# r-papso/carca-replication

Measured on AMD Instinct MI355X. Metric: scored users/sec (1+100 candidates), CARCA eval forward, higher is better.
Workload: dtype f32

## Files before the change

### carca_replication_amd/_lib.py

```python
from __future__ import annotations

import ctypes as C
import hashlib
import os
import shutil
import subprocess
import threading

_HERE = os.path.dirname(os.path.abspath(__file__))
_CSRC = os.path.join(_HERE, "csrc")
_INCLUDE = os.path.join(os.path.dirname(_HERE), "include")
LIB_PATH = os.path.join(_HERE, "libcarca_hip.so")
_STAMP = LIB_PATH + ".srchash"
SOURCES = ["api.hip", "gemm.hip", "gemm_wgrad.hip", "gemm_split.hip", "gemm_stream.hip", "wgrad_cu.hip", "decoders.hip", "batch_build.hip", "embed.hip", "sa_block.hip", "sa_eval.hip", "cross_score.hip", "cross_stream.hip", "loss_metrics.hip", "backward.hip", "block_bwd.hip", "row_chain.hip", "optim.hip", "recommend.hip", "rank.hip", "knn_catalogue.hip",
           "catalogue_xent.hip", "feat_dedup.hip", "sampled_xent.hip", "sampled_bce.hip", "similar_items.hip"]
HEADERS = ["carca_common.h", "gemm_host.h", "attn_common.h", "gemm_epilogue.h", "cross_fold.h", "recommend_common.h", "catalogue_select.h",
           "catalogue_sweep.h", "xent_tile.h", "xent_stage.h"]

MAX_SEGS = 4
MAX_GROUPS = 3
MAX_L = 64

_lock = threading.Lock()
_lib = None
# ... 294 lines not shown
    "carca_sa_block_eval": (_i, [_fp, _i, _fp, _fp, _i, _i, _i, _i, _i, C.POINTER(SaWeights), _i, _i, _fp]),
    "carca_cross_score_fwd": (_i, [_fp, _i, _fp, _fp, C.POINTER(TargetGroup), _i, _i, _i, _i, _i, _i,
                                   C.POINTER(CaWeights), _i, _i, C.POINTER(CaSave), C.POINTER(Dropout), _fp]),
    "carca_dropout_fwd": (_i, [_fp, _i, _i, _i, C.POINTER(Dropout), _fp, _fp]),
    "carca_mask_mul": (_i, [_fp, _i, _fp, _i, _f, _fp, _i, _i, _i, _i, _fp]),
    "carca_layernorm_bwd": (_i, [_fp, _i, _fp, _i, _fp, _i, _i, _fp, _i, _fp, _i, _i, _fp, _fp, _fp]),
    "carca_embed_scatter": (_i, [_fp, _i, _fp, _i, _i, _f, _fp, _fp]),
    "carca_colsum": (_i, [_fp, _i, _i, _i, _fp, _fp, _i, _fp, _fp]),
    "carca_sa_attn_bwd": (_i, [_fp, _fp, _fp, _fp, _i, _fp, _fp, _fp, _fp, _i, _i, _i, _i, _fp, _f, _fp]),
    "carca_cross_attn_bwd": (_i, [_fp, _fp, _fp, C.POINTER(CrossBwdGroup), _i, _fp, _fp, _fp, _fp, _i, _i, _i, _i, _i,
                                  _f, _fp]),
    "carca_unpack_grads": (_i, [C.POINTER(PackDesc), _i, _i, _fp]),
    "carca_forward": (_i, [C.POINTER(ForwardDesc), C.POINTER(_fp), _fp]),
    "carca_event_create": (_i, [C.POINTER(_fp)]),
    "carca_event_destroy": (_i, [_fp]),
    "carca_event_elapsed_ms": (_i, [_fp, _fp, C.POINTER(C.c_float)]),
    "carca_stream_wait_event": (_i, [_fp, _fp]),
    "carca_bce_fwd": (_i, [_fp, _fp, _fp, _i, _f, _fp, _fp, _fp, _fp, _fp]),
    "carca_rank_metrics": (_i, [_fp, _i, _i, _i, _fp, _fp, _fp, _fp]),
    "carca_eval_metrics": (_i, [_fp, _fp, _fp, _i, _i, _i, _f, _fp, _fp]),
    "carca_layernorm_fwd": (_i, [_fp, _i, _fp, _i, _i, _i, _fp, _fp, _fp]),
    "carca_dot_score_fwd": (_i, [_fp, _i, _fp, _i, _fp, _i, _i, _i, _i, _i, _i, _fp]),
    "carca_dot_score_bwd": (_i, [_fp, _i, _fp, _i, _fp, _fp, _fp, _i, _fp, _i, _i, _i, _i, _i, _i, _i, _fp]),
    "carca_slot_decay_scale": (_i, [_fp, _i, _fp, _i, _i, _i, _i, _f, _fp]),
    "carca_l2norm_fwd": (_i, [_fp, _i, _fp, _i, _i, _i, _fp]),
    "carca_l2norm_bwd": (_i, [_fp, _i, _fp, _i, _fp, _i, _i, _i, _fp]),
    "carca_add_positions": (_i, [_fp, _i, _fp, _fp, _i, _i, _i, _i, _fp]),
    "carca_mha_core": (_i, [_fp, _i, _fp, _fp, _i, _fp, _fp, _i, _i, _i, _i, _i, _i, _i, _fp, _i, _fp, _fp]),
    "carca_mha_core_bwd": (_i, [_fp, _i, _fp, _fp, _i, _fp, _fp, _i, _i, _i, _i, _i, _i, _i, _fp, _i, _fp, _fp, _fp, _fp,
                                _fp]),
    "carca_gemm_rows_log": (_i, [C.c_char_p, _i]),
    "carca_feat_dedup_rows_multiplied": (C.c_longlong, []),
    "carca_feat_dedup_rows_computed": (C.c_longlong, []),
    "carca_feat_cache_arm": (_i, [C.POINTER(FeatCache)]),
    "carca_get_tuning": (_i, [_i]),
    "carca_mha_core_drop": (_i, [_fp, _i, _fp, _fp, _i, _fp, _fp, _i, _i, _i, _i, _i, _i, _i, _fp, _i, _fp, C.POINTER(Dropout),
                                 _fp, _fp]),
    "carca_mha_core_bwd_drop": (_i, [_fp, _i, _fp, _fp, _i, _fp, _fp, _i, _i, _i, _i, _i, _i, _i, _fp, _i, _fp, _fp, _fp, _fp,
                                     _fp, C.c_float, _fp]),
    "carca_knn_score": (_i, [_fp, C.c_int64, _fp, C.c_int64, _fp, _fp, _i, _fp, _i, _i, _i, _i, _fp]),
    "carca_sa_block_bwd_workspace": (C.c_size_t, [_i, _i, _i, _i]),
    "carca_sa_block_bwd": (_i, [C.POINTER(SaBwdDesc), C.POINTER(WgradDesc), C.POINTER(_i), _fp]),
    "carca_cross_score_bwd_workspace": (C.c_size_t, [_i, _i, _i, _i, C.POINTER(C.c_int32), _i]),
    "carca_cross_score_bwd": (_i, [C.POINTER(CrossBwdDesc), C.POINTER(WgradDesc), C.POINTER(_i), _fp]),
    "carca_embed_bwd_workspace": (C.c_size_t, [C.POINTER(C.c_int32), _i, _i, _i]),
    "carca_embed_bwd": (_i, [C.POINTER(EmbedBwdDesc), _fp]),
    "carca_early_event_recorded": (_i, []),
    "carca_adam_step": (_i, [C.POINTER(AdamTensor), _i, C.c_double, C.c_double, C.c_double, C.c_double, C.c_double, _i,
                        _fp]),
    "carca_mark_rows": (_i, [_fp, C.c_int64, _fp, C.c_int64, _fp]),
    "carca_zero_rows": (_i, [_fp, C.c_int64, _i, C.POINTER(_fp), C.POINTER(C.c_int64), _i, _fp]),
    "carca_concat_ids": (_i, [C.POINTER(_fp), C.POINTER(C.c_int64), _i, _fp, _fp]),
    "carca_build_eval_batch": (_i, [_fp, _fp, _fp, _fp, _i, _i, _i, _i, _i, _i, _i, _i, C.c_uint64, _fp, _fp, _fp, _fp, _fp,
                                    _fp]),
    "carca_recommend": (_i, [C.POINTER(RecommendDesc), _fp]),
    "carca_rank_items": (_i, [C.POINTER(RankDesc), _fp]),
    "carca_recommend_among": (_i, [C.POINTER(RecommendDesc), C.POINTER(Candidates), _fp]),
    "carca_rank_items_among": (_i, [C.POINTER(RankDesc), C.POINTER(Candidates), _fp]),
    "carca_knn_recommend": (_i, [C.POINTER(KnnRecommendDesc), _fp]),
    "carca_knn_rank_items": (_i, [C.POINTER(KnnRankDesc), _fp]),
    "carca_row_rnorm": (_i, [_fp, _i, _i, _i, _fp, _fp]),
    "carca_similar_items": (_i, [C.POINTER(SimilarDesc), C.POINTER(Candidates), _fp]),
    "carca_catalogue_xent_fwd": (_i, [C.POINTER(CatalogueXentDesc), _fp]),
    "carca_catalogue_xent_bwd": (_i, [C.POINTER(CatalogueXentDesc), _fp]),
    "carca_sampled_xent_fwd": (_i, [C.POINTER(SampledXentDesc), _fp]),
    "carca_sampled_xent_bwd": (_i, [C.POINTER(SampledXentDesc), _fp]),
# ... 48 lines not shown
```

### carca_replication_amd/csrc/carca_common.h

```cpp
#pragma once
#include <hip/hip_runtime.h>
#include <stdint.h>

#include "../../include/carca_hip.h"

typedef float f32x4 __attribute__((ext_vector_type(4)));
typedef float f32x16 __attribute__((ext_vector_type(16)));
typedef float f32x4_u __attribute__((ext_vector_type(4), aligned(4)));

#define CARCA_WAVE 64

typedef unsigned u32x4 __attribute__((ext_vector_type(4)));
__device__ __forceinline__ __amdgpu_buffer_rsrc_t carca_rsrc(const void* base) {
  return __builtin_amdgcn_make_buffer_rsrc(const_cast<void*>(base), 0, -1, 0x00020000);
}
__device__ __forceinline__ f32x4 gload4(const float* base, int elem_off) {
  const u32x4 v = __builtin_amdgcn_raw_buffer_load_b128(carca_rsrc(base), elem_off * 4, 0, 0);
  f32x4 f = {__uint_as_float(v[0]), __uint_as_float(v[1]), __uint_as_float(v[2]), __uint_as_float(v[3])};
  return f;
}
__device__ __forceinline__ f32x4 gload4s(const float* base, int lane_elem_off, int uniform_elem_off) {
  const u32x4 v = __builtin_amdgcn_raw_buffer_load_b128(carca_rsrc(base), lane_elem_off * 4, uniform_elem_off * 4, 0);
  f32x4 f = {__uint_as_float(v[0]), __uint_as_float(v[1]), __uint_as_float(v[2]), __uint_as_float(v[3])};
  return f;
// ... 130 lines not shown
      for (int i = 0; i < RIF; ++i) v[i] = c < ga.d ? src[i][c] : 0.f;
#pragma unroll
      for (int i = 0; i < RIF; ++i)
        if (c < ga.d && row0 + i < ga.total_rows) ga.zq[(size_t)(row0 + i) * ga.ldz + c] = v[i] * ga.scale;
    }
  }
}

template <int BYTES>
__device__ __forceinline__ void carca_warm_kernargs() {
  typedef const __attribute__((address_space(4))) int* karg_ptr;
  karg_ptr ka = (karg_ptr)__builtin_amdgcn_kernarg_segment_ptr();
  int w = 0;
#pragma unroll
  for (int i = 0; i < (BYTES + 63) / 64; ++i) w ^= ka[i * 16];
  asm volatile("" ::"s"(w));
}

enum { CARCA_TUNE_GEMM_VARIANT = 0, CARCA_TUNE_ATTN_VARIANT = 1, CARCA_TUNE_WGRAD_SLOTS = 2,
       CARCA_TUNE_WGRAD_PLAIN_STORE = 3,
       CARCA_TUNE_WGRAD_MIN_CHUNKS = 4,
       CARCA_TUNE_WGRAD_GROUP_SLOTS = 5,
       CARCA_TUNE_N96S_DIAG = 5,
       CARCA_TUNE_ROUND1_PATHS = 6,
       CARCA_TUNE_SCORE_LAYOUT = 7,
       CARCA_TUNE_DETERMINISTIC = 8,
       CARCA_TUNE_STAMPS = 9, CARCA_TUNE_CU_CAP = 10, CARCA_TUNE_SK_DON = 11, CARCA_TUNE_SK_SPIN_LOG2 = 12,
       CARCA_TUNE_SK_WITHHOLD = 13, CARCA_TUNE_XS_OPT = 14, CARCA_TUNE_DIAG = 15, CARCA_TUNE_SPLIT_GEMM = 16,
       CARCA_TUNE_SKC_OV_TEAM = 17,
       CARCA_TUNE_SKC_OV_LONE = 18,
       CARCA_TUNE_SKC_MIN_STEPS = 19,
       CARCA_TUNE_FEAT_DEDUP = 20,
       CARCA_TUNE_FEAT_CACHE = 21,
       CARCA_TUNE_COUNT = 24 };
enum {
  CARCA_GV_AUTO = 0,
  CARCA_GV_TILED = 1,
  CARCA_GV_PER_CU = 2,
  CARCA_GV_PER_CU_STAMPS = 3,
  CARCA_GV_NO_BUFFER_LOADS = 4,
  CARCA_GV_WGRAD_TILED = 5,
  CARCA_GV_NO_GROUP = 6,
  CARCA_GV_PER_CU_128 = 7,
  CARCA_GV_NO_PASSENGER = 8,
  CARCA_GV_WIDE64 = 9,
  CARCA_GV_WIDE64_PF2 = 10,
  CARCA_GV_N96 = 11,
  CARCA_GV_NO_N96 = 12,
  CARCA_GV_WGRAD_EQUAL_ITEMS = 13,
  CARCA_GV_WGRAD_ATOMIC_FLUSH = 14,
  CARCA_GV_NO_STREAM_K = 15,
  CARCA_GV_WGRAD_FLAT_GROUPS = 16,
  CARCA_GV_GATHER_ROW_PER_WAVE = 18,
  CARCA_GV_OWN_GATHER = 19,
  CARCA_GV_WPART_ATOMICS = 19,
  CARCA_GV_SPLIT_NO_DMA = 21,
  CARCA_GV_WGRAD_NO_COMPACT = 22,
  CARCA_GV_SK_EVERY_ROW = 23,
  CARCA_GV_NO_CUS = 24,
  CARCA_GV_CUS = 25,
  CARCA_GV_NO_N96S = 26,
  CARCA_GV_N96S = 27,
  CARCA_GV_NO_STREAM_K_NO_PASSENGER = 158,
};
int carca_tuning(int key);
int carca_num_cus();
bool carca_stream_capturing(hipStream_t stream);
void* carca_stream_scratch(hipStream_t stream, int tag, size_t bytes, size_t zero_bytes = 0, bool* fresh = nullptr);
enum { CARCA_SCRATCH_SK = 1, CARCA_SCRATCH_WPART = 2, CARCA_SCRATCH_WTAB = 3, CARCA_SCRATCH_SPLITW = 4, CARCA_SCRATCH_SKC = 5,
       CARCA_SCRATCH_SKC_PART = 6, CARCA_SCRATCH_RECOMMEND = 7, CARCA_SCRATCH_RANK = 8,
       CARCA_SCRATCH_KNN = 9, CARCA_SCRATCH_DEDUP_HASH = 10, CARCA_SCRATCH_DEDUP = 11, CARCA_SCRATCH_SIMILAR = 12 };
void* carca_capture_alloc(hipStream_t stream, size_t bytes, bool host_mapped, void** device_view, size_t zero_bytes = 0);
void carca_arm_launch_events(void* start, void* stop);
bool carca_take_launch_events(hipEvent_t* start, hipEvent_t* stop);
bool carca_take_feat_cache(CarcaFeatCache* out);
struct CarcaGemmDesc;
void carca_rows_log(const char* kernel, const CarcaGemmDesc* d, int grid);
int carca_gemm_rows_split_try(const CarcaGemmDesc* desc, hipStream_t stream);
int carca_gemm_rows_stream_try(const CarcaGemmDesc* desc, bool fits32, hipStream_t stream);
int carca_gemm_rows_n96s_try(const CarcaGemmDesc* desc, bool fits32, hipStream_t stream);
int carca_gemm_rows_passenger(const CarcaGemmDesc* desc, const CarcaGatherArgs* ga, int* rode, void* stream);
struct CarcaDedupRun {
  CarcaGemmDesc d;
  int nseg, R, vec, vec2, hbits;
  int row0[CARCA_MAX_SEGS + 1];
  unsigned hmask;
  int* key;
  unsigned* val;
  int *slot, *rep, *flag;
  float* P;
  float* wcb;
  int ldp;
  CarcaFeatCache cache;
  int *need, *pub, *cnt;
};
int carca_feat_dedup_prepare(const CarcaGemmDesc* desc, hipStream_t stream, CarcaDedupRun* run);
int carca_feat_dedup_plan(const CarcaDedupRun* run, hipStream_t stream, hipEvent_t start);
int carca_feat_dedup_expand(const CarcaDedupRun* run, hipStream_t stream, hipEvent_t stop);
int carca_gemm_rows_feat_dedup(const CarcaGemmDesc* desc, void* stream);
int* carca_kernel_error_word();
struct CarcaRowSeg;
int carca_embed_joint_ztab(const CarcaRowSeg* segs, int nseg, int d, int g, const float* joint_w, const float* joint_b,
                           const float* pos, const float* zq, int ld_e, const float* z_table, int ld_z_table, void* stream);
int carca_embed_scatter_segs(const float* const* dz, int ld_dz, const int32_t* const* ids, const int* rows, int nseg,
                             int d, float scale, float* d_items, void* stream);
int carca_sa_ffn_chain_bwd(const float* dy, const float* h1, const float* r, const float* w2_t, const float* w1_t,
                           const float* ln2_w, int rows, int d, int dpi, int residual, float* dh1pre, float* dr,
                           float* g_ln2_w, float* g_ln2_b, void* stream);
int carca_sa_input_chain_bwd(const float* dqh, const float* dkh, const float* dvh, const float* dr, const float* x_in,
                             const float* wq_t, const float* wk_t, const float* wv_t, const float* ln1_w, int rows, int d,
                             int dpi, int residual, float* dx, float* g_ln1_w, float* g_ln1_b, void* stream);
unsigned long long* carca_debug_buffer();
#define CARCA_CHECK_ARG(cond, ...)            \
  do {                                        \
    if (!(cond)) {                            \
      carca_set_error(__VA_ARGS__);           \
      return CARCA_ERR_BADARG;                \
    }                                         \
  } while (0)
#define CARCA_CHECK_SUPPORTED(cond, ...)      \
  do {                                        \
    if (!(cond)) {                            \
      carca_set_error(__VA_ARGS__);           \
      return CARCA_ERR_UNSUPPORTED;           \
    }                                         \
  } while (0)
#define CARCA_LAUNCH_CHECK()                                               \
// ... 8 lines not shown
```

### carca_replication_amd/csrc/feat_dedup.hip

```cpp
#include <hip/hip_ext.h>

#include <vector>

#include "carca_common.h"
#include "../../include/carca_hip.h"

namespace {

constexpr int EXP_ROWS = 16;
constexpr int EXP_MAX_N = 1024;
constexpr int EXP_MAX_K1 = 8;
constexpr int EXP_WB4 = ((EXP_MAX_K1 + 1) * EXP_MAX_N / 4 + 255) / 256;
__host__ __device__ inline int exp_wb_floats(int K1, int N) { return ((K1 + 1) * N + 3) / 4 * 4; }

__device__ __forceinline__ int dd_seg(const CarcaDedupRun& a, int g) {
  int s = 0;
#pragma unroll
  for (int i = 1; i < CARCA_MAX_SEGS; ++i)
    if (i < a.nseg && g >= a.row0[i]) s = i;
  return s;
}
__device__ __forceinline__ const float* dd_a0_row(const CarcaDedupRun& a, int s, int r) {
  const CarcaGemmSeg& sg = a.d.seg[s];
  if (sg.a0_gather) return sg.a0 + (size_t)sg.ids[r] * a.d.lda0;
  if (sg.a0_bstride) return sg.a0 + (size_t)(r / sg.T) * sg.a0_bstride + (size_t)(r % sg.T) * a.d.lda0;
  return sg.a0 + (size_t)r * a.d.lda0;
}

__global__ __launch_bounds__(256) void dedup_insert_kernel(const CarcaDedupRun a) {
  const int g = blockIdx.x * 256 + threadIdx.x;
  {
    const int N = a.d.N, K1 = a.d.K1, nw = exp_wb_floats(K1, N);
    for (int i = g; i < nw; i += gridDim.x * 256) {
      const int k = i / N, n = i - k * N;
      a.wcb[i] = k < K1 ? a.d.bt1[(size_t)n * a.d.ldb1 + k] : (k == K1 && a.d.bias ? a.d.bias[n] : 0.f);
    }
  }
  if (g == 0 && a.cnt) a.cnt[0] = 0;
  if (g >= a.R) return;
  const int s = dd_seg(a, g);
  const int id = a.d.seg[s].ids[g - a.row0[s]];
  int h = -1;
  if (id != 0) {
    unsigned hh = ((unsigned)id * 0x9E3779B1u) >> (32 - a.hbits);
    for (;;) {
      const int k = atomicCAS(&a.key[hh], 0, id);
      if (k == 0 || k == id) break;
      hh = (hh + 1) & a.hmask;
    }
    atomicMax(&a.val[hh], 0xFFFFFFFFu - (unsigned)g);
    h = (int)hh;
  }
  a.slot[g] = h;
}

template <bool VEC>
__device__ __forceinline__ bool dd_rows_differ(const unsigned* p, const unsigned* q, const int K, const int lane) {
  bool diff = false;
  if constexpr (VEC) {
    typedef unsigned u4 __attribute__((ext_vector_type(4)));
    for (int k0 = 0; k0 < K && !diff; k0 += 1024) {
      u4 x[4], y[4];
#pragma unroll
      for (int u = 0; u < 4; ++u) {
        const int k = k0 + (u * 64 + lane) * 4;
        x[u] = k < K ? *reinterpret_cast<const u4*>(p + k) : u4{0, 0, 0, 0};
        y[u] = k < K ? *reinterpret_cast<const u4*>(q + k) : u4{0, 0, 0, 0};
      }
      bool d = false;
#pragma unroll
      for (int u = 0; u < 4; ++u) d = d || x[u][0] != y[u][0] || x[u][1] != y[u][1] || x[u][2] != y[u][2] || x[u][3] != y[u][3];
      diff = __ballot(d) != 0;
    }
  } else {
    for (int k0 = 0; k0 < K && !diff; k0 += 256) {
      bool d = false;
#pragma unroll
      for (int u = 0; u < 4; ++u) {
        const int k = k0 + u * 64 + lane;
        if (k < K) d = d || p[k] != q[k];
      }
      diff = __ballot(d) != 0;
    }
  }
  return diff;
}

template <bool VEC>
__global__ __launch_bounds__(256) void dedup_resolve_kernel(const CarcaDedupRun a) {
  const int lane = threadIdx.x & 63;
  const int g = blockIdx.x * 4 + __builtin_amdgcn_readfirstlane((int)threadIdx.x >> 6);
  if (g >= a.R) return;
  const int h = a.slot[g];
  const bool cache = a.cache.state != nullptr;
  if (h < 0) {
    if (lane == 0) {
      a.rep[g] = -1;
      a.flag[g] = 0;
      if (cache) {
        a.need[g] = 0;
        a.pub[g] = 0;
      }
    }
    return;
  }
  const int r0 = (int)(0xFFFFFFFFu - a.val[h]);
  const int s = dd_seg(a, g);
  const CarcaGemmSeg& sg = a.d.seg[s];
  int ci = 0;
  bool filled = false, hit = false, from_table = false;
  if (cache) {
    const int id = __builtin_amdgcn_readfirstlane(a.key[h]);
    from_table = sg.a0_gather && sg.a0 == a.cache.table;
    if (id > 0 && id < a.cache.n_rows && (a.cache.a_c || from_table)) {
      ci = id;
      filled = a.cache.state[id] == 1;
    }
    if (filled) {
      if (a.cache.a_c) {
        const unsigned* p = reinterpret_cast<const unsigned*>(dd_a0_row(a, s, g - a.row0[s]));
        const unsigned* q = reinterpret_cast<const unsigned*>(a.cache.a_c + (size_t)ci * a.cache.ld_a);
        hit = !dd_rows_differ<VEC>(p, q, a.d.K0, lane);
      } else {
        hit = true;
      }
    }
  }
  bool merge = false;
  if (!hit && r0 != g) {
    const int t = dd_seg(a, r0);
    const CarcaGemmSeg& tg = a.d.seg[t];
    merge = sg.a0_gather && tg.a0_gather && sg.a0 == tg.a0;
    if (!merge) {
      const unsigned* p = reinterpret_cast<const unsigned*>(dd_a0_row(a, s, g - a.row0[s]));
      const unsigned* q = reinterpret_cast<const unsigned*>(dd_a0_row(a, t, r0 - a.row0[t]));
      merge = !dd_rows_differ<VEC>(p, q, a.d.K0, lane);
    }
  }
  if (lane == 0) {
    a.rep[g] = hit ? -2 - ci : (merge ? r0 : g);
    a.flag[g] = hit ? (r0 == g ? 1 : 0) : (merge ? 0 : 1);
    if (cache) {
      const int need = !hit && !merge;
      a.need[g] = need;
      a.pub[g] = r0 == g && ci > 0 && !filled ? ci : 0;
      if (need) atomicAdd(a.cnt, 1);
    }
    if (r0 != g) a.slot[g] = -1;
  }
}

struct DdRowSeg {
  const float* a1;
  float* c;
  long a1_bstride;
  int T, r;
};
__device__ __forceinline__ DdRowSeg dd_row_seg(const CarcaDedupRun& a, int g) {
  DdRowSeg o{a.d.seg[0].a1, a.d.seg[0].c, a.d.seg[0].a1_bstride, a.d.seg[0].T, g};
#pragma unroll
  for (int i = 1; i < CARCA_MAX_SEGS; ++i)
    if (i < a.nseg && g >= a.row0[i]) o = DdRowSeg{a.d.seg[i].a1, a.d.seg[i].c, a.d.seg[i].a1_bstride, a.d.seg[i].T, g - a.row0[i]};
  return o;
}

template <int VW>
__global__ __launch_bounds__(256) void dedup_expand_kernel(const CarcaDedupRun a) {
  typedef float vec __attribute__((ext_vector_type(VW)));
  typedef float f4 __attribute__((ext_vector_type(4)));
  extern __shared__ f4 exp_lds[];
  carca_warm_kernargs<sizeof(CarcaDedupRun)>();
  const int N = a.d.N, K1 = a.d.K1, nw4 = exp_wb_floats(K1, N) / 4;
  float* Ws = reinterpret_cast<float*>(exp_lds);
  float* cxs = Ws + nw4 * 4;
  int* reps = reinterpret_cast<int*>(cxs + EXP_ROWS * EXP_MAX_K1);
  int* pubs = reps + EXP_ROWS;
  const bool cache = a.cache.state != nullptr;
  const int tid = threadIdx.x, g0 = blockIdx.x * EXP_ROWS;
  f4 w[EXP_WB4];
  const f4* wcb4 = reinterpret_cast<const f4*>(a.wcb);
#pragma unroll
  for (int j = 0; j < EXP_WB4; ++j) {
    const int i = tid + j * 256;
    if (i < nw4) w[j] = wcb4[i];
  }
  if (tid < EXP_ROWS * EXP_MAX_K1) {
    const int row = tid / EXP_MAX_K1, k = tid % EXP_MAX_K1, g = g0 + row;
    float cv = 0.f;
    if (g < a.R && k < K1) {
      const DdRowSeg sg = dd_row_seg(a, g);
      const float* cr = sg.a1_bstride ? sg.a1 + (size_t)(sg.r / sg.T) * sg.a1_bstride + (size_t)(sg.r % sg.T) * a.d.lda1
                                      : sg.a1 + (size_t)sg.r * a.d.lda1;
      cv = cr[k];
    }
    cxs[tid] = cv;
  } else if (tid < EXP_ROWS * EXP_MAX_K1 + EXP_ROWS) {
    const int row = tid - EXP_ROWS * EXP_MAX_K1, g = g0 + row;
    int u = -2, pb = 0;
    if (g < a.R) {
      u = a.rep[g];
      if (cache) pb = a.pub[g];
      const int h = a.slot[g];
      if (h >= 0) {
        a.key[h] = 0;
        a.val[h] = 0u;
      }
    }
    reps[row] = u;
    pubs[row] = pb;
  }
#pragma unroll
  for (int j = 0; j < EXP_WB4; ++j) {
    const int i = tid + j * 256;
    if (i < nw4) exp_lds[i] = w[j];
  }
  __syncthreads();
  const int lane = tid & 63, wave = __builtin_amdgcn_readfirstlane(tid >> 6);
  constexpr int RW = EXP_ROWS / 4, CH = 4;
  const int nv = N / VW;
  int u[RW], pb[RW];
  vec* crow[RW];
  const vec* prow[RW];
#pragma unroll
  for (int i = 0; i < RW; ++i) {
    const int row = wave * RW + i;
    u[i] = __builtin_amdgcn_readfirstlane(reps[row]);
    pb[i] = __builtin_amdgcn_readfirstlane(pubs[row]);
    const DdRowSeg sg = dd_row_seg(a, min(g0 + row, a.R - 1));
    crow[i] = reinterpret_cast<vec*>(sg.c + (size_t)sg.r * a.d.ldc);
    prow[i] = reinterpret_cast<const vec*>(u[i] < -2 ? a.cache.p_c + (size_t)(-2 - u[i]) * a.cache.ld_p
                                                    : a.P + (size_t)max(u[i], 0) * a.ldp);
  }
  const vec* Wv = reinterpret_cast<const vec*>(Ws);
  for (int c0 = 0; c0 < nv; c0 += CH * 64) {
    vec v[RW][CH];
#pragma unroll
    for (int i = 0; i < RW; ++i) {
#pragma unroll
// ... 28 lines not shown
    for (int c = 0; c < CH; ++c) {
      const int p = c0 + c * 64 + lane;
      const vec b = Wv[K1 * nv + min(p, nv - 1)];
#pragma unroll
      for (int i = 0; i < RW; ++i)
        if (u[i] != -2 && p < nv) crow[i][p] = u[i] != -1 ? v[i][c] + b : vec(0.f);
    }
  }
  if (cache) {
#pragma unroll 1
    for (int i = 0; i < RW; ++i) {
      if (pb[i] <= 0) continue;
      if (a.cache.a_c) {
        const int g = g0 + wave * RW + i, s = dd_seg(a, g);
        const float* src = dd_a0_row(a, s, g - a.row0[s]);
        float* dst = a.cache.a_c + (size_t)pb[i] * a.cache.ld_a;
        if (a.vec) {
          const f4* s4 = reinterpret_cast<const f4*>(src);
          f4* d4 = reinterpret_cast<f4*>(dst);
          for (int k = lane; k < a.d.K0 / 4; k += 64) d4[k] = s4[k];
        } else {
          for (int k = lane; k < a.d.K0; k += 64) dst[k] = src[k];
        }
      }
      if (lane == 0) a.cache.state[pb[i]] = 1;
    }
  }
}

struct DdLast {
  hipStream_t stream;
  size_t bytes, flag_off, need_off;
  int R;
};
thread_local DdLast g_dd_last{nullptr, 0, 0, 0, 0};

}

int carca_feat_dedup_prepare(const CarcaGemmDesc* desc, hipStream_t stream, CarcaDedupRun* run) {
  const CarcaGemmDesc& D = *desc;
  if (D.K1 > EXP_MAX_K1 || D.N > EXP_MAX_N || D.ncols_out != D.N || (D.alpha != 0.f && D.alpha != 1.f) || !D.mask_rows ||
      (D.K1 > 0 && !D.bt1))
    return 1;
  CarcaDedupRun& a = *run;
  a = CarcaDedupRun{};
  a.d = D;
  a.nseg = D.nseg;
  long R = 0;
  bool vec = D.K0 % 4 == 0 && D.lda0 % 4 == 0;
  for (int s = 0; s < D.nseg; ++s) {
    const CarcaGemmSeg& sg = D.seg[s];
    if (!sg.ids || sg.add || sg.gate || sg.rowscale || sg.add_pos) return 1;
    if (a.d.seg[s].T < 1) a.d.seg[s].T = 1;
    vec = vec && ((uintptr_t)sg.a0 & 15) == 0 && sg.a0_bstride % 4 == 0;
    a.row0[s] = (int)R;
    R += sg.rows;
  }
  for (int s = D.nseg; s <= CARCA_MAX_SEGS; ++s) a.row0[s] = (int)R;
  if (R < 1 || R > (1l << 28)) return 1;
  a.R = (int)R;
  a.vec = vec ? 1 : 0;
  int hb = 12;
  while ((1l << hb) < 2 * R) ++hb;
  a.hbits = hb;
  a.hmask = (1u << hb) - 1;
  a.ldp = D.N;
  bool vec2 = D.N % 2 == 0 && D.ldc % 2 == 0;
  for (int s = 0; s < D.nseg; ++s) vec2 = vec2 && ((uintptr_t)D.seg[s].c & 7) == 0;
  a.vec2 = vec2 ? 1 : 0;
  const bool cap = carca_stream_capturing(stream);
  bool knobs = false;
  for (int k : {CARCA_TUNE_GEMM_VARIANT, CARCA_TUNE_STAMPS, CARCA_TUNE_CU_CAP, CARCA_TUNE_SK_DON, CARCA_TUNE_SK_SPIN_LOG2,
                CARCA_TUNE_SK_WITHHOLD, CARCA_TUNE_DIAG, CARCA_TUNE_SKC_OV_TEAM, CARCA_TUNE_SKC_OV_LONE,
                CARCA_TUNE_SKC_MIN_STEPS})
    knobs = knobs || carca_tuning(k) != 0;
  CarcaFeatCache fc;
  const bool cached = carca_take_feat_cache(&fc) && !cap && !knobs && carca_tuning(CARCA_TUNE_FEAT_CACHE) != 1 &&
                      fc.ld_p >= D.N && (!fc.a_c || fc.ld_a >= D.K0);
  if (cached) {
    a.cache = fc;
    if (fc.a_c && (((uintptr_t)fc.a_c & 15) != 0 || fc.ld_a % 4 != 0)) a.vec = 0;
    if (((uintptr_t)fc.p_c & 7) != 0 || fc.ld_p % 2 != 0) a.vec2 = 0;
  }
  const size_t hbytes = (size_t)2 * sizeof(int) << hb;
  const size_t ibytes = ((size_t)(cached ? 5 * R + 1 : 3 * R) * sizeof(int) + 255) / 256 * 256;
  const size_t wbytes = ((size_t)exp_wb_floats(D.K1, D.N) * sizeof(float) + 255) / 256 * 256;
  const size_t bytes = ibytes + wbytes + (size_t)R * a.ldp * sizeof(float);
  char* ht = (char*)(cap ? carca_capture_alloc(stream, hbytes, false, nullptr, hbytes)
                         : carca_stream_scratch(stream, CARCA_SCRATCH_DEDUP_HASH, hbytes, hbytes));
  char* buf = (char*)(cap ? carca_capture_alloc(stream, bytes, false, nullptr)
                          : carca_stream_scratch(stream, CARCA_SCRATCH_DEDUP, bytes));
  if (!ht || !buf) return (int)hipErrorOutOfMemory;
  a.key = (int*)ht;
  a.val = (unsigned*)(ht + ((size_t)sizeof(int) << hb));
  a.slot = (int*)buf;
  a.rep = a.slot + R;
  a.flag = a.rep + R;
  if (cached) {
    a.need = a.flag + R;
    a.pub = a.need + R;
    a.cnt = a.pub + R;
  }
  a.wcb = (float*)(buf + ibytes);
  a.P = (float*)(buf + ibytes + wbytes);
  g_dd_last = cap ? DdLast{nullptr, 0, 0, 0, 0}
                  : DdLast{stream, bytes, (size_t)2 * R * sizeof(int), (size_t)(cached ? 3 : 2) * R * sizeof(int), a.R};
  return CARCA_OK;
}

int carca_feat_dedup_plan(const CarcaDedupRun* run, hipStream_t stream, hipEvent_t start) {
  const CarcaDedupRun& a = *run;
  const dim3 gi((a.R + 255) / 256), gr((a.R + 3) / 4);
  if (start)
    hipExtLaunchKernelGGL(dedup_insert_kernel, gi, dim3(256), 0, stream, start, nullptr, 0, a);
  else
    hipLaunchKernelGGL(dedup_insert_kernel, gi, dim3(256), 0, stream, a);
  CARCA_LAUNCH_CHECK();
  if (a.vec)
    hipLaunchKernelGGL(dedup_resolve_kernel<true>, gr, dim3(256), 0, stream, a);
  else
    hipLaunchKernelGGL(dedup_resolve_kernel<false>, gr, dim3(256), 0, stream, a);
  CARCA_LAUNCH_CHECK();
  return CARCA_OK;
}

int carca_feat_dedup_expand(const CarcaDedupRun* run, hipStream_t stream, hipEvent_t stop) {
  const CarcaDedupRun& a = *run;
  const dim3 ge((a.R + EXP_ROWS - 1) / EXP_ROWS);
  const size_t lds = ((size_t)exp_wb_floats(a.d.K1, a.d.N) + EXP_ROWS * EXP_MAX_K1 + 2 * EXP_ROWS) * sizeof(float);
  auto kern = a.vec2 ? dedup_expand_kernel<2> : dedup_expand_kernel<1>;
  if (stop)
    hipExtLaunchKernelGGL(kern, ge, dim3(256), lds, stream, nullptr, stop, 0, a);
  else
    hipLaunchKernelGGL(kern, ge, dim3(256), lds, stream, a);
  CARCA_LAUNCH_CHECK();
  return CARCA_OK;
}

static long long dd_count_last(size_t DdLast::*off) {
  const DdLast l = g_dd_last;
  if (!l.R) return -1;
  const char* buf = (const char*)carca_stream_scratch(l.stream, CARCA_SCRATCH_DEDUP, l.bytes);
  if (!buf) return -1;
  std::vector<int> flag(l.R);
  if (hipMemcpyAsync(flag.data(), buf + l.*off, (size_t)l.R * sizeof(int), hipMemcpyDeviceToHost, l.stream) != hipSuccess ||
      hipStreamSynchronize(l.stream) != hipSuccess)
    return -1;
  long long n = 0;
  for (int f : flag) n += f != 0;
  return n;
}

extern "C" long long carca_feat_dedup_rows_multiplied(void) { return dd_count_last(&DdLast::flag_off); }
extern "C" long long carca_feat_dedup_rows_computed(void) { return dd_count_last(&DdLast::need_off); }
```

### carca_replication_amd/csrc/gemm.hip

```cpp
#include "gemm_host.h"
#include <type_traits>
#include <vector>
#include "../../include/carca_hip.h"
#include "gemm_epilogue.h"
#include <cstring>
#include <string>

static thread_local std::string g_rows_log;
static thread_local bool g_rows_log_on = false;
void carca_rows_log(const char* kernel, const CarcaGemmDesc* d, int grid) {
  if (!g_rows_log_on || g_rows_log.size() > 60000) return;
  long rows = 0;
  for (int s = 0; s < d->nseg; ++s) rows += d->seg[s].rows;
  char buf[256];
  snprintf(buf, sizeof(buf), "%s rows=%ld N=%d K=%d grid=%d;", kernel, rows, d->N, d->K0 + d->K1, grid);
  g_rows_log += buf;
}
extern "C" int carca_gemm_rows_log(char* out, int cap) {
  if (!out) {
    g_rows_log.clear();
    g_rows_log_on = cap != 0;
    return 0;
  }
  const int n = (int)std::min<size_t>(g_rows_log.size(), cap > 0 ? (size_t)cap - 1 : 0);
// ... 1588 lines not shown
    g.has_pas = 1;
    g.pas = *pas;
    ++grid;
    if (rode) *rode = 1;
  }
  if (g_rows_log_on) carca_rows_log(TN == 4 ? "gemm_rows_cu_kernel<0,4>" : "gemm_rows_cu_kernel<0,3>", desc, grid);
  carca_launch(gemm_rows_cu_kernel<DBG, TN>, dim3(grid), dim3(768), 0, stream, true, g);
  CARCA_LAUNCH_CHECK();
  return CARCA_OK;
}

int* g_sk_err_host = nullptr;
int* g_sk_err_dev = nullptr;

int* carca_kernel_error_word() {
  if (!g_sk_err_host) {
    if (hipHostMalloc((void**)&g_sk_err_host, sizeof(int), hipHostMallocMapped | hipHostMallocPortable) != hipSuccess) {
      (void)hipGetLastError();
      return nullptr;
    }
    *g_sk_err_host = 0;
    if (hipHostGetDevicePointer((void**)&g_sk_err_dev, g_sk_err_host, 0) != hipSuccess) g_sk_err_dev = nullptr;
  }
  return g_sk_err_dev;
}
static int sk_check_error_word() {
  if (g_sk_err_host && *(volatile int*)g_sk_err_host == 3) {
    *(volatile int*)g_sk_err_host = 0;
    carca_set_error("gemm_wgrad: an EARLIER gemm_wgrad_cu_kernel launch met a group whose range touches more k blocks than it "
                    "has partial-tile slots (that tile's gradient is wrong): a launcher bug -- carca_set_tuning(0, 14) "
                    "selects the atomic flush");
    return CARCA_ERR_UNSUPPORTED;
  }
  if (g_sk_err_host && *(volatile int*)g_sk_err_host == 2) {
    *(volatile int*)g_sk_err_host = 0;
    carca_set_error("gemm_rows: an EARLIER gemm_rows_skc_kernel launch met a stretch of more row blocks than its lists hold "
                    "(its output is wrong): a launcher bug -- carca_set_tuning(0, 23) selects the kernel over every row");
    return CARCA_ERR_UNSUPPORTED;
  }
  if (g_sk_err_host && *(volatile int*)g_sk_err_host != 0) {
    *(volatile int*)g_sk_err_host = 0;
    carca_set_error("gemm_rows: an EARLIER stream-K launch gave up waiting for a partial tile (its output is wrong): "
                    "were its workgroups not all resident?  carca_set_tuning(0, 15) selects the kernel without the hand-over");
    return CARCA_ERR_UNSUPPORTED;
  }
  return CARCA_OK;
}
extern "C" int carca_poll_errors(void) { return sk_check_error_word(); }

static int sk_handover_setup(GemmDev& g) {
  g.sk_err = carca_kernel_error_word();
  if (!g_sk_err_host) return 1;
  if (int rc = sk_check_error_word()) return rc;
  const int lg = carca_tuning(CARCA_TUNE_SK_SPIN_LOG2);
  g.sk_spin = 1u << (lg > 0 && lg < 31 ? lg : 23);
  g.sk_withhold = carca_tuning(CARCA_TUNE_SK_WITHHOLD);
  return CARCA_OK;
}

static int launch_gemm_rows_sk(const CarcaGemmDesc* desc, hipStream_t stream, const CarcaGatherArgs* pas, int* rode) {
  const int variant = carca_tuning(CARCA_TUNE_GEMM_VARIANT);
  if (variant == CARCA_GV_NO_STREAM_K || variant == CARCA_GV_NO_STREAM_K_NO_PASSENGER) return 1;
  const int ncb = (desc->ncols_out + 95) / 96, nfull = ncb - 1;
  if (ncb < 2 || desc->ncols_out != desc->N) return 1;
  const int rem = desc->N - 96 * nfull, xc = rem - 64;
  if (xc < 1 || xc > 2) return 1;
// ... 335 lines not shown
```

### carca_replication_amd/ops.py

```python
from __future__ import annotations

import ctypes as C
import functools
import math
from dataclasses import dataclass
from typing import Iterable, List, Optional, Sequence, Tuple

import torch
from torch import Tensor

from . import _lib
from ._lib import CarcaHipError


_stage_events = None


def set_stage_events(ev) -> None:
    global _stage_events
    _stage_events = ev


_fused_events = None

# ... 1095 lines not shown

def capture_bytes(scope: int) -> int:
    return int(_lib.load().carca_capture_bytes(C.c_ulonglong(scope)))


def capture_release(scope: int) -> None:
    if scope:
        _lib.check(_lib.load().carca_capture_release(C.c_ulonglong(scope)), "capture_release")


TUNE_SPLIT_GEMM = 16
SPLIT_GEMM_MODES = {"fp32": 0, "bf16x3": 1, "fp16x2": 2}
_split_mode = 0


def gemm_rows_log(on: Optional[bool] = None) -> str:
    lib = _lib.load()
    if on is not None:
        lib.carca_gemm_rows_log(None, int(bool(on)))
        return ""
    buf = C.create_string_buffer(65536)
    lib.carca_gemm_rows_log(buf, len(buf))
    return buf.value.decode()


def feat_dedup_rows_multiplied() -> int:
    return int(_lib.load().carca_feat_dedup_rows_multiplied())


def feat_dedup_rows_computed() -> int:
    return int(_lib.load().carca_feat_dedup_rows_computed())


TUNE_FEAT_CACHE = 21


def get_tuning(key: int) -> int:
    return int(_lib.load().carca_get_tuning(int(key)))


def set_feature_gemm_precision(mode: str, force: bool = False) -> None:
    global _split_mode
    set_tuning(TUNE_SPLIT_GEMM, SPLIT_GEMM_MODES[mode] | (16 if force and SPLIT_GEMM_MODES[mode] else 0))
    _split_mode = SPLIT_GEMM_MODES[mode]
    if _split_mode == 0:
        _lib.check(_lib.load().carca_split_bind(None, None, 0, 0, 0), "split_bind")


def feature_gemm_mode() -> int:
    return _split_mode


def split_launch_count() -> int:
    return int(_lib.load().carca_split_launch_count())


def split_pack(w: Tensor, K0: int, mode: int) -> Tensor:
    w = _f32(w.detach())
    _need_cuda(w)
    lib = _lib.load()
    N = w.shape[0]
    out = torch.empty(int(lib.carca_split_bytes(N, int(K0), int(mode))), dtype=torch.uint8, device=w.device)
    _lib.check(lib.carca_split_pack(w.data_ptr(), w.stride(0), int(K0), N, int(mode), out.data_ptr(), _stream()), "split_pack")
    return out


def split_bind(w: Optional[Tensor], planes: Optional[Tensor], mode: int = 0, K0: int = 0) -> None:
# ... 351 lines not shown
```

### include/carca_hip.h

```cpp
#ifndef CARCA_HIP_H
#define CARCA_HIP_H

#include <stdint.h>

#ifdef __cplusplus
extern "C" {
#endif

#define CARCA_ABI_VERSION 3
#define CARCA_OK 0
#define CARCA_ERR_UNSUPPORTED (-1)
#define CARCA_ERR_BADARG (-2)

#define CARCA_MAX_SEGS 4
#define CARCA_MAX_GROUPS 3
#define CARCA_MAX_L 64
#define CARCA_EMBED_GATHER 1
#define CARCA_EMBED_FEAT 2
#define CARCA_EMBED_JOINT 4
#define CARCA_EMBED_ALL 7
#define CARCA_EMBED_DEDUP 8

int carca_abi_version(void);
int carca_set_tuning(int key, int value);
// ... 180 lines not shown
  const int32_t* ids;
  float* dqh;
  float* dlogit;
  const uint8_t* m_attn;
  int32_t N;
  int32_t ld_y;
} CarcaCrossBwdGroup;
int carca_cross_attn_bwd(const float* kh, const float* vh, const int32_t* p_ids, const CarcaCrossBwdGroup* groups,
                         int ngroups, const float* ffn_w_pad, float* dkh, float* dvh, float* d_ffn_w_pad, int B, int L,
                         int d, int H, int training, float drop_scale, void* stream);
int carca_dropout_fwd(float* x, int rows, int cols, int ld, const CarcaDropout* drop, uint8_t* mask, void* stream);
int carca_mask_mul(const float* x, int ld_x, const uint8_t* mask, int ld_m, float scale, float* out, int ld_out,
                   int rows, int cols, int ncols_out, void* stream);
int carca_layernorm_fwd(const float* x, int ldx, float* y, int ldy, int rows, int d, const float* w, const float* b,
                        void* stream);
int carca_dot_score_fwd(const float* p, int ldp, const float* o, int ldo, float* y, int B, int L, int T, int d,
                        int slotwise, int link, void* stream);
int carca_dot_score_bwd(const float* p, int ldp, const float* o, int ldo, const float* y, const float* dy, float* dp,
                        int ld_dp, float* d_o, int ld_do, int B, int L, int T, int d, int slotwise, int link,
                        void* stream);
int carca_slot_decay_scale(const float* x, int ldx, float* out, int ldo, int B, int L, int d, float gamma, void* stream);
int carca_l2norm_fwd(const float* x, int ldx, float* y, int ldy, int rows, int d, void* stream);
int carca_l2norm_bwd(const float* x, int ldx, const float* dy, int ld_dy, float* dx, int ld_dx, int rows, int d,
                     void* stream);
int carca_knn_score(const float* p_a, int64_t p_bstride, const float* o_a, int64_t o_bstride, const int32_t* p_x,
                    const int32_t* o_x, int table_rows, float* y, int B, int L, int T, int F, void* stream);
int carca_add_positions(const float* x, int ldx, const float* pos, float* out, int ldo, int B, int T, int d, void* stream);
int carca_mha_core(const float* q, int ldq, const float* k, const float* v, int ldk, const int32_t* q_ids,
                   const int32_t* k_ids, int B, int Tq, int Tk, int d, int H, int has_causal, int causal, float* out,
                   int ldo, float* w_out , void* stream);
int carca_gemm_rows_log(char* out , int cap);
long long carca_feat_dedup_rows_multiplied(void);
long long carca_feat_dedup_rows_computed(void);
typedef struct {
  float* p_c;
  float* a_c;
  int32_t* state;
  const float* table;
  int32_t n_rows, ld_p, ld_a;
} CarcaFeatCache;
int carca_feat_cache_arm(const CarcaFeatCache* cache );
int carca_get_tuning(int key);
int carca_mha_core_drop(const float* q, int ldq, const float* k, const float* v, int ldk, const int32_t* q_ids,
                        const int32_t* k_ids, int B, int Tq, int Tk, int d, int H, int has_causal, int causal, float* out,
                        int ldo, float* w_out , const CarcaDropout* drop , uint8_t* keep_out ,
                        void* stream);
int carca_mha_core_bwd(const float* q, int ldq, const float* k, const float* v, int ldk, const int32_t* q_ids,
                       const int32_t* k_ids, int B, int Tq, int Tk, int d, int H, int has_causal, int causal,
                       const float* d_out , int ldo, const float* d_w , float* dq, float* dk, float* dv,
                       void* stream);
int carca_mha_core_bwd_drop(const float* q, int ldq, const float* k, const float* v, int ldk, const int32_t* q_ids,
                            const int32_t* k_ids, int B, int Tq, int Tk, int d, int H, int has_causal, int causal,
                            const float* d_out , int ldo, const float* d_w , float* dq, float* dk,
                            float* dv, const uint8_t* keep , float keep_scale, void* stream);
int carca_unpack_grads(const CarcaPackDesc* descs, int n, int accumulate, void* stream);

typedef struct CarcaSaBwdDesc {
  int32_t B, L, d, H, residual;
  float drop_p;
  const int32_t* ids;
  const float* dy;
  const float *x_in, *qn, *qh, *kh, *vh, *r, *s2, *h1;
  const uint8_t *m_attn, *m_ffn2;
  const float *wq_t, *wk_t, *wv_t;
  const float *w1_t, *w2_t;
  const float *ln1_w, *ln2_w;
// ... 347 lines not shown
```

Measured before the change: 703,100.

## Group cached-row dedup compares so one wave checks four rows against the cache

The insert kernel now records each row's rank in its hash slot and keeps a short per-slot member list. In the resolve kernel, when the feature cache is filled, a leader wave loads the cached feature row once and compares up to four member rows against it in one interleaved pass, with the other members returning early. The intent is to cut redundant reads of the cached row and the number of waves doing full-length compares on repeated items. In exchange it adds an atomic counter and member-list writes per row, extra workspace, an error word for out-of-range members, and a tuning switch that restores the per-row compare.

Result: faster. 774,000, median of 6 (+10.1%).

```diff
diff --git a/carca_replication_amd/_lib.py b/carca_replication_amd/_lib.py
--- a/carca_replication_amd/_lib.py
+++ b/carca_replication_amd/_lib.py
@@ -350,6 +350,7 @@
     "carca_gemm_rows_log": (_i, [C.c_char_p, _i]),
     "carca_feat_dedup_rows_multiplied": (C.c_longlong, []),
     "carca_feat_dedup_rows_computed": (C.c_longlong, []),
+    "carca_feat_dedup_rows_grouped": (C.c_longlong, []),
     "carca_feat_cache_arm": (_i, [C.POINTER(FeatCache)]),
     "carca_get_tuning": (_i, [_i]),
     "carca_mha_core_drop": (_i, [_fp, _i, _fp, _fp, _i, _fp, _fp, _i, _i, _i, _i, _i, _i, _i, _fp, _i, _fp, C.POINTER(Dropout),
diff --git a/carca_replication_amd/csrc/carca_common.h b/carca_replication_amd/csrc/carca_common.h
--- a/carca_replication_amd/csrc/carca_common.h
+++ b/carca_replication_amd/csrc/carca_common.h
@@ -186,6 +186,7 @@
        CARCA_TUNE_SKC_MIN_STEPS = 19,
        CARCA_TUNE_FEAT_DEDUP = 20,
        CARCA_TUNE_FEAT_CACHE = 21,
+       CARCA_TUNE_DEDUP_SOLO = 22,
        CARCA_TUNE_COUNT = 24 };
 enum {
   CARCA_GV_AUTO = 0,
@@ -247,6 +248,9 @@
   int ldp;
   CarcaFeatCache cache;
   int *need, *pub, *cnt;
+  int *rank, *grp, *cnt_slot, *mem;
+  int solo;
+  int* err;
 };
 int carca_feat_dedup_prepare(const CarcaGemmDesc* desc, hipStream_t stream, CarcaDedupRun* run);
 int carca_feat_dedup_plan(const CarcaDedupRun* run, hipStream_t stream, hipEvent_t start);
diff --git a/carca_replication_amd/csrc/feat_dedup.hip b/carca_replication_amd/csrc/feat_dedup.hip
--- a/carca_replication_amd/csrc/feat_dedup.hip
+++ b/carca_replication_amd/csrc/feat_dedup.hip
@@ -12,6 +12,9 @@
 constexpr int EXP_MAX_K1 = 8;
 constexpr int EXP_WB4 = ((EXP_MAX_K1 + 1) * EXP_MAX_N / 4 + 255) / 256;
 __host__ __device__ inline int exp_wb_floats(int K1, int N) { return ((K1 + 1) * N + 3) / 4 * 4; }
+constexpr int DD_LIST = 16;
+constexpr int DD_GROUP = 4;
+static_assert(DD_LIST % DD_GROUP == 0 && DD_GROUP <= 8, "a leader's ranks stay inside the list");
 
 __device__ __forceinline__ int dd_seg(const CarcaDedupRun& a, int g) {
   int s = 0;
@@ -50,6 +53,11 @@
     }
     atomicMax(&a.val[hh], 0xFFFFFFFFu - (unsigned)g);
     h = (int)hh;
+    if (a.cnt_slot) {
+      const int k = atomicAdd(&a.cnt_slot[hh], 1);
+      a.rank[g] = k;
+      if (k < DD_LIST) a.mem[(size_t)hh * DD_LIST + k] = g;
+    }
   }
   a.slot[g] = h;
 }
@@ -87,6 +95,85 @@
 }
 
 template <bool VEC>
+__device__ __forceinline__ unsigned dd_group_differ(const unsigned* const (&p)[DD_GROUP], const int n, const unsigned* q,
+                                                    const int K, const int lane) {
+  unsigned diff = 0;
+  const unsigned all = (1u << n) - 1u;
+  if constexpr (VEC) {
+    typedef unsigned u4 __attribute__((ext_vector_type(4)));
+    constexpr int RU = 2;
+    for (int k0 = 0; k0 < K && diff != all; k0 += RU * 256) {
+      u4 y[RU], x[DD_GROUP][RU];
+#pragma unroll
+      for (int u = 0; u < RU; ++u) {
+        const int k = k0 + (u * 64 + lane) * 4;
+        y[u] = k < K ? *reinterpret_cast<const u4*>(q + k) : u4{0, 0, 0, 0};
+      }
+#pragma unroll
+      for (int j = 0; j < DD_GROUP; ++j) {
+        const bool on = j < n && !((diff >> j) & 1u);
+#pragma unroll
+        for (int u = 0; u < RU; ++u) {
+          const int k = k0 + (u * 64 + lane) * 4;
+          x[j][u] = on && k < K ? __builtin_nontemporal_load(reinterpret_cast<const u4*>(p[j] + k)) : u4{0, 0, 0, 0};
+        }
+      }
+#pragma unroll
+      for (int j = 0; j < DD_GROUP; ++j) {
+        const bool on = j < n && !((diff >> j) & 1u);
+        bool d = false;
+#pragma unroll
+        for (int u = 0; u < RU; ++u)
+          d = d || x[j][u][0] != y[u][0] || x[j][u][1] != y[u][1] || x[j][u][2] != y[u][2] || x[j][u][3] != y[u][3];
+        if (on && __ballot(d) != 0) diff |= 1u << j;
+      }
+    }
+  } else {
+    for (int k0 = 0; k0 < K && diff != all; k0 += 256) {
+      bool d[DD_GROUP];
+#pragma unroll
+      for (int j = 0; j < DD_GROUP; ++j) d[j] = false;
+#pragma unroll
+      for (int u = 0; u < 4; ++u) {
+        const int k = k0 + u * 64 + lane;
+        if (k < K) {
+          const unsigned y = q[k];
+#pragma unroll
+          for (int j = 0; j < DD_GROUP; ++j)
+            if (j < n && !((diff >> j) & 1u)) d[j] = d[j] || p[j][k] != y;
+        }
+      }
+#pragma unroll
+      for (int j = 0; j < DD_GROUP; ++j)
+        if (j < n && __ballot(d[j]) != 0) diff |= 1u << j;
+    }
+  }
+  return diff;
+}
+
+template <bool VEC>
+__device__ __forceinline__ bool dd_merges(const CarcaDedupRun& a, const int g, const int r0, const int lane) {
+  const int s = dd_seg(a, g), t = dd_seg(a, r0);
+  const CarcaGemmSeg &sg = a.d.seg[s], &tg = a.d.seg[t];
+  if (sg.a0_gather && tg.a0_gather && sg.a0 == tg.a0) return true;
+  const unsigned* p = reinterpret_cast<const unsigned*>(dd_a0_row(a, s, g - a.row0[s]));
+  const unsigned* q = reinterpret_cast<const unsigned*>(dd_a0_row(a, t, r0 - a.row0[t]));
+  return !dd_rows_differ<VEC>(p, q, a.d.K0, lane);
+}
+
+__device__ __forceinline__ void dd_write_row(const CarcaDedupRun& a, const int g, const int r0, const int ci, const bool filled,
+                                             const bool hit, const bool merge) {
+  a.rep[g] = hit ? -2 - ci : (merge ? r0 : g);
+  a.flag[g] = hit ? (r0 == g ? 1 : 0) : (merge ? 0 : 1);
+  if (a.cache.state) {
+    const int need = !hit && !merge;
+    a.need[g] = need;
+    a.pub[g] = r0 == g && ci > 0 && !filled ? ci : 0;
+    if (need) atomicAdd(a.cnt, 1);
+  }
+}
+
+template <bool VEC, bool GROUPS>
 __global__ __launch_bounds__(256) void dedup_resolve_kernel(const CarcaDedupRun a) {
   const int lane = threadIdx.x & 63;
   const int g = blockIdx.x * 4 + __builtin_amdgcn_readfirstlane((int)threadIdx.x >> 6);
@@ -101,9 +188,12 @@
         a.need[g] = 0;
         a.pub[g] = 0;
       }
+      if (a.grp) a.grp[g] = 0;
     }
     return;
   }
+  int rk = DD_LIST;
+  if constexpr (GROUPS) rk = a.rank[g];
   const int r0 = (int)(0xFFFFFFFFu - a.val[h]);
   const int s = dd_seg(a, g);
   const CarcaGemmSeg& sg = a.d.seg[s];
@@ -116,6 +206,43 @@
       ci = id;
       filled = a.cache.state[id] == 1;
     }
+    if (GROUPS && filled && rk < DD_LIST) {
+      if (rk % DD_GROUP == 0) {
+        const int n = min(min(a.cnt_slot[h], DD_LIST) - rk, DD_GROUP);
+        int m[DD_GROUP];
+        const unsigned* p[DD_GROUP];
+        bool bad = false;
+#pragma unroll
+        for (int j = 0; j < DD_GROUP; ++j) {
+          m[j] = j > 0 && j < n ? __builtin_amdgcn_readfirstlane(a.mem[(size_t)h * DD_LIST + rk + j]) : g;
+          if ((unsigned)m[j] >= (unsigned)a.R) {
+            bad = true;
+            m[j] = g;
+          }
+          const int t = dd_seg(a, m[j]);
+          p[j] = reinterpret_cast<const unsigned*>(dd_a0_row(a, t, m[j] - a.row0[t]));
+        }
+        if (bad && lane == 0 && a.err) *a.err = 4;
+        const unsigned* q = reinterpret_cast<const unsigned*>(a.cache.a_c + (size_t)ci * a.cache.ld_a);
+        const unsigned diff = dd_group_differ<VEC>(p, n, q, a.d.K0, lane);
+#pragma unroll 1
+        for (int j = 0; j < n; ++j) {
+          int mj = g;
+#pragma unroll
+          for (int i = 1; i < DD_GROUP; ++i)
+            if (j == i) mj = m[i];
+          const bool hj = !((diff >> j) & 1u);
+          bool merge = false;
+          if (!hj && r0 != mj) merge = dd_merges<VEC>(a, mj, r0, lane);
+          if (lane == 0) {
+            dd_write_row(a, mj, r0, ci, true, hj, merge);
+            a.grp[mj] = 1;
+          }
+        }
+      }
+      if (lane == 0 && r0 != g) a.slot[g] = -1;
+      return;
+    }
     if (filled) {
       if (a.cache.a_c) {
         const unsigned* p = reinterpret_cast<const unsigned*>(dd_a0_row(a, s, g - a.row0[s]));
@@ -127,25 +254,10 @@
     }
   }
   bool merge = false;
-  if (!hit && r0 != g) {
-    const int t = dd_seg(a, r0);
-    const CarcaGemmSeg& tg = a.d.seg[t];
-    merge = sg.a0_gather && tg.a0_gather && sg.a0 == tg.a0;
-    if (!merge) {
-      const unsigned* p = reinterpret_cast<const unsigned*>(dd_a0_row(a, s, g - a.row0[s]));
-      const unsigned* q = reinterpret_cast<const unsigned*>(dd_a0_row(a, t, r0 - a.row0[t]));
-      merge = !dd_rows_differ<VEC>(p, q, a.d.K0, lane);
-    }
-  }
+  if (!hit && r0 != g) merge = dd_merges<VEC>(a, g, r0, lane);
   if (lane == 0) {
-    a.rep[g] = hit ? -2 - ci : (merge ? r0 : g);
-    a.flag[g] = hit ? (r0 == g ? 1 : 0) : (merge ? 0 : 1);
-    if (cache) {
-      const int need = !hit && !merge;
-      a.need[g] = need;
-      a.pub[g] = r0 == g && ci > 0 && !filled ? ci : 0;
-      if (need) atomicAdd(a.cnt, 1);
-    }
+    dd_write_row(a, g, r0, ci, filled, hit, merge);
+    if (a.grp) a.grp[g] = 0;
     if (r0 != g) a.slot[g] = -1;
   }
 }
@@ -204,6 +316,7 @@
       if (h >= 0) {
         a.key[h] = 0;
         a.val[h] = 0u;
+        if (a.cnt_slot) a.cnt_slot[h] = 0;
       }
     }
     reps[row] = u;
@@ -298,8 +411,9 @@
   hipStream_t stream;
   size_t bytes, flag_off, need_off;
   int R;
+  size_t grp_off;
 };
-thread_local DdLast g_dd_last{nullptr, 0, 0, 0, 0};
+thread_local DdLast g_dd_last{nullptr, 0, 0, 0, 0, 0};
 
 }
 
@@ -348,8 +462,11 @@
     if (fc.a_c && (((uintptr_t)fc.a_c & 15) != 0 || fc.ld_a % 4 != 0)) a.vec = 0;
     if (((uintptr_t)fc.p_c & 7) != 0 || fc.ld_p % 2 != 0) a.vec2 = 0;
   }
-  const size_t hbytes = (size_t)2 * sizeof(int) << hb;
-  const size_t ibytes = ((size_t)(cached ? 5 * R + 1 : 3 * R) * sizeof(int) + 255) / 256 * 256;
+  const bool ranked = cached && fc.a_c != nullptr;
+  a.solo = carca_tuning(CARCA_TUNE_DEDUP_SOLO) == 1 ? 1 : 0;
+  const size_t hbytes = (size_t)3 * sizeof(int) << hb;
+  const size_t nints = (size_t)(cached ? 5 * R + 1 : 3 * R) + (ranked ? (size_t)2 * R + ((size_t)DD_LIST << hb) : 0);
+  const size_t ibytes = (nints * sizeof(int) + 255) / 256 * 256;
   const size_t wbytes = ((size_t)exp_wb_floats(D.K1, D.N) * sizeof(float) + 255) / 256 * 256;
   const size_t bytes = ibytes + wbytes + (size_t)R * a.ldp * sizeof(float);
   char* ht = (char*)(cap ? carca_capture_alloc(stream, hbytes, false, nullptr, hbytes)
@@ -367,10 +484,18 @@
     a.pub = a.need + R;
     a.cnt = a.pub + R;
   }
+  if (ranked) {
+    a.err = carca_kernel_error_word();
+    a.cnt_slot = (int*)(ht + ((size_t)2 * sizeof(int) << hb));
+    a.rank = a.cnt + 1;
+    a.grp = a.rank + R;
+    a.mem = a.grp + R;
+  }
   a.wcb = (float*)(buf + ibytes);
   a.P = (float*)(buf + ibytes + wbytes);
   g_dd_last = cap ? DdLast{nullptr, 0, 0, 0, 0}
-                  : DdLast{stream, bytes, (size_t)2 * R * sizeof(int), (size_t)(cached ? 3 : 2) * R * sizeof(int), a.R};
+                  : DdLast{stream, bytes, (size_t)2 * R * sizeof(int), (size_t)(cached ? 3 : 2) * R * sizeof(int), a.R,
+                           ranked ? (size_t)(6 * R + 1) * sizeof(int) : 0};
   return CARCA_OK;
 }
 
@@ -382,10 +507,10 @@
   else
     hipLaunchKernelGGL(dedup_insert_kernel, gi, dim3(256), 0, stream, a);
   CARCA_LAUNCH_CHECK();
-  if (a.vec)
-    hipLaunchKernelGGL(dedup_resolve_kernel<true>, gr, dim3(256), 0, stream, a);
-  else
-    hipLaunchKernelGGL(dedup_resolve_kernel<false>, gr, dim3(256), 0, stream, a);
+  const bool groups = a.rank != nullptr && !a.solo;
+  auto kern = a.vec ? (groups ? dedup_resolve_kernel<true, true> : dedup_resolve_kernel<true, false>)
+                    : (groups ? dedup_resolve_kernel<false, true> : dedup_resolve_kernel<false, false>);
+  hipLaunchKernelGGL(kern, gr, dim3(256), 0, stream, a);
   CARCA_LAUNCH_CHECK();
   return CARCA_OK;
 }
@@ -419,3 +544,6 @@
 
 extern "C" long long carca_feat_dedup_rows_multiplied(void) { return dd_count_last(&DdLast::flag_off); }
 extern "C" long long carca_feat_dedup_rows_computed(void) { return dd_count_last(&DdLast::need_off); }
+extern "C" long long carca_feat_dedup_rows_grouped(void) {
+  return g_dd_last.grp_off ? dd_count_last(&DdLast::grp_off) : 0;
+}
diff --git a/carca_replication_amd/csrc/gemm.hip b/carca_replication_amd/csrc/gemm.hip
--- a/carca_replication_amd/csrc/gemm.hip
+++ b/carca_replication_amd/csrc/gemm.hip
@@ -1644,6 +1644,12 @@
                     "selects the atomic flush");
     return CARCA_ERR_UNSUPPORTED;
   }
+  if (g_sk_err_host && *(volatile int*)g_sk_err_host == 4) {
+    *(volatile int*)g_sk_err_host = 0;
+    carca_set_error("feat_dedup: an EARLIER dedup_resolve_kernel launch met a row list that names a row outside its batch "
+                    "(rows of that item keep no outputs): a bug -- carca_set_tuning(22, 1) selects the per-row compare");
+    return CARCA_ERR_UNSUPPORTED;
+  }
   if (g_sk_err_host && *(volatile int*)g_sk_err_host == 2) {
     *(volatile int*)g_sk_err_host = 0;
     carca_set_error("gemm_rows: an EARLIER gemm_rows_skc_kernel launch met a stretch of more row blocks than its lists hold "
diff --git a/carca_replication_amd/ops.py b/carca_replication_amd/ops.py
--- a/carca_replication_amd/ops.py
+++ b/carca_replication_amd/ops.py
@@ -1151,7 +1151,12 @@
     return int(_lib.load().carca_feat_dedup_rows_computed())
 
 
+def feat_dedup_rows_grouped() -> int:
+    return int(_lib.load().carca_feat_dedup_rows_grouped())
+
+
 TUNE_FEAT_CACHE = 21
+TUNE_DEDUP_SOLO = 22
 
 
 def get_tuning(key: int) -> int:
diff --git a/include/carca_hip.h b/include/carca_hip.h
--- a/include/carca_hip.h
+++ b/include/carca_hip.h
@@ -236,6 +236,7 @@
 int carca_gemm_rows_log(char* out , int cap);
 long long carca_feat_dedup_rows_multiplied(void);
 long long carca_feat_dedup_rows_computed(void);
+long long carca_feat_dedup_rows_grouped(void);
 typedef struct {
   float* p_c;
   float* a_c;
```
